# Opendigitalradio/ODR-AudioEnc

Hardware: AMD Instinct MI355X
Metric: real-time stereo DAB MP2 streams sustained (frames/s) @128 kbps/48 kHz (higher is better)
Workload: dtype f64; 1 GPU; 4096 streams/GPU x 48 kHz stereo (mode 's') x 128 kbps, psy 1, full encode (BASELINE configs[1]), 32 frames/stream/step; streams_per_gpu=4096, parallelism=streams sharded over 1 GPU(s), no data-path collective

## Files before the change

odr-audioenc_amd/csrc/mp2_pack.h:

```cpp
#ifndef MP2_WAVE_PARTS
#error "include mp2_wave.h"
#endif
struct TlFrameOut { uint8_t *bytes; uint32_t *words; uint8_t *scfcrc; };
template <int PSY, int NCH = 0>
TL_FN void tl_encode_frame(TlMainLds &w, const TlTables *TL_RESTRICT T, const TlBlockShared *TL_RESTRICT B,
                           const TlConfig *TL_RESTRICT C, const TlPsyOut *TL_RESTRICT PO,
                           const TlPcmView &pv, int xpad_len, const TlFrameOut &fo,
                           const double *TL_RESTRICT enw_s, const TlPackTables *TL_RESTRICT K, int padding, TlTaps *taps, long long *sp)
{
    constexpr int FB = TlMainLds::kFbBatch;
    const int nch = NCH ? NCH : C->nch, sblimit = C->sblimit;
    PA(double, smp, 36);
    PA(int, scf, 3);

    TL_STAMP(sp, 0);
    TL_PRIO2(TL_PS_FB);
    tl_filterbank(w, B, enw_s, nch, smp);

    TL_STAMP(sp, 1);
    TL_PRIO2(1);
#if !defined(TL_EMULATE) && TL_ENC_LEVEL >= 5
    for (int b = 0; b < 36; b++) TL_KEEP(smp[b]);
    scf[0] = scf[1] = scf[2] = 0;
#endif
    PV(int, a_ln); PV(int, a_nbal);
    TL_LANES_BEGIN
// ... 433 lines not shown
            int bytepos = i < xpad_len - 2 ? xstart + i : lg_frame - 2 + (i - (xpad_len - 2));
            tl_put_bits(frame, bytepos * 8, w.xpad[i], 8);
        }
    }
    TL_LANES_END

    } else {
        TL_LANES_BEGIN
        if (lane < 4) w.ncentre[lane] = 0;
        TL_LANES_END
    }
    if (taps) {
        TL_LANES_BEGIN
        const int c = lane & 1, sb = lane >> 1;
        taps->smr[c][sb] = (c < nch && (C->psy != 1 || sb < sblimit)) ? w.smr[c][sb] : 0.0;
        taps->scfsi[c][sb] = w.scfsi[c][sb]; taps->bit_alloc[c][sb] = w.balloc[c][sb];
        for (int gr = 0; gr < 3; gr++) taps->scalar[c][gr][sb] = w.scf[c][gr][sb];
        if (lane == 0) { taps->adb_left = adb_left; taps->mode = mode; taps->mode_ext = mode_ext; taps->jsbound = jsbound; taps->crc16 = (int)crc16; }
        if (lane < 4) taps->scfcrc[lane] = lane < C->dab_ext ? (uint8_t)w.ncentre[lane] : 0;
        TL_LANES_END
    }

    TL_STAMP(sp, 6);
    const int nwords = (lg_frame + 3) >> 2;
    TL_LANES_BEGIN
    for (int i = lane; i < nwords; i += 64) {
        if (fo.words) fo.words[i] = frame[i];
        else {
            const uint32_t le = tl_bswap(frame[i]);
            const int rem = lg_frame - 4 * i;
            if (rem >= 4) ((uint32_t *)fo.bytes)[i] = le;
            else for (int b = 0; b < rem; b++) fo.bytes[4 * i + b] = (uint8_t)(le >> (8 * b));
        }
    }
    if (lane < 4) fo.scfcrc[lane] = lane < C->dab_ext ? (uint8_t)w.ncentre[lane] : 0;
    TL_LANES_END
    TL_PRIO2(0);
    TL_STAMP(sp, 7);
}

template <int PSY>
TL_FN void tl_encode_pair(TlMainLds &w, const TlBlockShared *TL_RESTRICT B, const TlConfig *TL_RESTRICT C, const TlPsyOut *const (&PO)[2],
                          const int (&xpad_len)[2], const uint8_t *const (&xpad_src)[2], const TlFrameOut (&fo)[2],
                          const double *TL_RESTRICT enw_s, const TlPackTables *TL_RESTRICT K, const int (&padding)[2])
{
    const int sblimit = C->sblimit;
    const int padpk = padding[0] | (padding[1] << 1);
    PA(double, smp, 36);
    PA(int, scf, 3);
    TL_PRIO2(TL_PS_FB);
    tl_filterbank(w, B, enw_s, 2, smp);
    TL_PRIO2(1);
    TL_LANES_BEGIN
    const int c = lane & 1, sb = lane >> 1;
    if (sb < sblimit) {
        unsigned lo = 63;
        for (int gr = 0; gr < 3; gr++) {
            double m = fabs(L(smp)[gr * 12 + 11]);
            for (int j = 10; j >= 0; j--) { double t = fabs(L(smp)[gr * 12 + j]); if (t > m) m = t; }
// ... 234 lines not shown
        const int u = lane >> 5, l5 = lane & 31;
        if (l5 < C->dab_ext) {
            const int grp = C->dab_ext - 1 - l5;
            const unsigned c8 = ((grp == 0 ? c8g[0] : grp == 1 ? c8g[1] : grp == 2 ? c8g[2] : c8g[3]) >> (16 * u)) & 0xffu;
            const int tail = (u ? lg_frame[1] : lg_frame[0]) - 2 - C->dab_ext;
            tl_put_bits(w.u.frame[u], (tail + l5) * 8, c8, 8);
            w.ncentre[4 * u + l5] = (int16_t)c8;
        }
        TL_LANES_END
    }
#pragma unroll
    for (int u = 0; u < 2; u++)
        if (xpad_len[u]) {
            const int xl = xpad_len[u], xstart = lg_frame[u] - C->dab_ext - xl;
            TL_LANES_BEGIN
            for (int i = lane; i < xl; i += 64) {
                const int bytepos = i < xl - 2 ? xstart + i : lg_frame[u] - 2 + (i - (xl - 2));
                tl_put_bits(w.u.frame[u], bytepos * 8, xpad_src[u][i], 8);
            }
            TL_LANES_END
        }
#pragma unroll
    for (int u = 0; u < 2; u++) {
        const int nwords = (lg_frame[u] + 3) >> 2;
        const uint32_t *frame = w.u.frame[u];
        TL_LANES_BEGIN
        for (int i = lane; i < nwords; i += 64) {
            if (fo[u].words) fo[u].words[i] = frame[i];
            else {
                const uint32_t le = tl_bswap(frame[i]);
                const int rem = lg_frame[u] - 4 * i;
                if (rem >= 4) ((uint32_t *)fo[u].bytes)[i] = le;
                else for (int b = 0; b < rem; b++) fo[u].bytes[4 * i + b] = (uint8_t)(le >> (8 * b));
            }
        }
        if (lane < 4) fo[u].scfcrc[lane] = lane < C->dab_ext ? (uint8_t)w.ncentre[4 * u + lane] : 0;
        TL_LANES_END
    }
    TL_PRIO2(0);
}
```

odr-audioenc_amd/csrc/mp2_types.h:

```cpp
#pragma once
#include <stdint.h>

#define TL_MAX_FRAME_BYTES 1728
#define TL_MAX_FRAME_WORDS (TL_MAX_FRAME_BYTES / 4)
#define TL_HIST 480
#define TL_MAX_XPAD 256

struct TlBlockShared {
    double dbtable[1002];
    double scalefactor[64];
    double snr_line[9][16];
    int16_t bits12_line[9][16];
    uint16_t qinfo_line[9][16];
    double dct_t[16][2][16];
    uint8_t sfpat[32];
    double scale_db[64];
};

struct TlPackTables {
    double qa[18], qb[18];
    double steps2n_f[18];
    int32_t steps[18];
    int32_t steps2n[18];
    uint16_t crc_xpow[512];
// ... 104 lines not shown
    const int32_t *stream_cfg;
    const int32_t *stream_list;
    TlStreamState *state;
    const int16_t *pcm;
    const uint8_t *xpad;
    const int32_t *xpad_len;
    uint8_t *out;
    int32_t *out_len;
    TlTaps *taps;
    long long *stamps;
    const TlPsy2Tables *psy2_tables;
    TlPsy2State *psy2_state;
    TlPsyOut *psy_out;
    uint8_t *scfcrc;
    uint32_t *newpend;
    uint8_t *padbits;
    double *newlag;
    int32_t *work;
    const int32_t *partner;
    const int32_t *chain_list;
    int32_t nstreams, nframes, out_stride, nlist;
    int32_t nchain, p2_nwhole, p2_k, p2_plen;
    int32_t psy2_flip, pad_;
};
```

odr-audioenc_amd/csrc/mp2_units.h:

```cpp
#ifndef MP2_WAVE_PARTS
#error "include mp2_wave.h"
#endif
TL_FN int tl_cfg_index(const TlLaunch &A, int s) { return A.stream_cfg ? A.stream_cfg[s] : 0; }
TL_FN int tl_slot_step(double &lag, double frac)
{
    if (frac == 0) return 0;
    if (lag > (frac - 1.0)) { lag -= frac; return 0; }
    lag += (1 - frac);
    return 1;
}
TL_FN void tl_slots_stream(const TlLaunch &A, int s)
{
    const double frac = A.configs[tl_cfg_index(A, s)].pad_frac;
    double lag = A.state[s].slot_lag;
    for (int f = 0; f < A.nframes; f++) A.padbits[(size_t)f * (size_t)A.nstreams + (size_t)s] = (uint8_t)tl_slot_step(lag, frac);
    A.newlag[s] = lag;
}

TL_FN TlPcmView tl_pcm_view(const TlLaunch &A, const TlStreamState *st, int s, int f)
{
    const size_t slot = (size_t)f * (size_t)A.nstreams + (size_t)s;
    TlPcmView pv;
    pv.cur[0] = A.pcm + slot * 2304; pv.cur[1] = pv.cur[0] + 1152;
    pv.hist[0] = f == 0 ? &st->hist[0][0] : A.pcm + (slot - (size_t)A.nstreams) * 2304 + (1152 - TL_HIST);
// ... 119 lines not shown
#pragma unroll
        for (int c = 0; c < 2; c++) {
            if (c >= nch) break;
            uint64_t *d = (uint64_t *)&w.u.fbk.pcm[c][0];
#pragma unroll
            for (int it = 0; it < HT; it++) if (64 * it + 64 <= HP || lane < HP - 64 * it) d[lane + 64 * it] = vh[c][it];
#pragma unroll
            for (int it = 0; it < CT; it++) if (64 * it + 64 <= CP || lane < CP - 64 * it) d[HP + lane + 64 * it] = vc[c][it];
        }
    }
    TL_LANES_END
}
TL_FN int tl_stage_xpad(TlMainLds &w, const TlLaunch &A, const TlConfig *C, size_t slot)
{
    if (!A.xpad_len) return 0;
    int xl = A.xpad_len[slot];
    if (xl < 2 || xl > TL_MAX_XPAD || xl > C->dab_length) xl = 0;
    TL_LANES_BEGIN
    for (int i = lane; i < xl; i += 64) w.xpad[i] = A.xpad[slot * TL_MAX_XPAD + i];
    TL_LANES_END
    return xl;
}

template <int PSY, int NCH = 0>
TL_FN void tl_main_unit(TlMainLds &w, const TlBlockShared *TL_RESTRICT B, const double *TL_RESTRICT enw_s, const TlPackTables *TL_RESTRICT K, const TlLaunch &A, int s, int f, int ci = -1)
{
    const TlConfig *C = &A.configs[ci >= 0 ? ci : TL_UNI_I(tl_cfg_index(A, s))];
    TlStreamState *st = &A.state[s];
    const size_t slot = (size_t)f * (size_t)A.nstreams + (size_t)s;
    const TlPcmView pv = tl_pcm_view(A, st, s, f);
#ifdef TL_NO_MAIN_STAMPS
    long long *sp = nullptr;
#else
    long long *sp = A.stamps ? A.stamps + slot * 32 : nullptr;
#endif
    TL_STAMP(sp, 31);
    tl_stage_pcm(w, pv, NCH ? NCH : C->nch);
    const int xl = tl_stage_xpad(w, A, C, slot);
    TlFrameOut fo;
    fo.bytes = f + 1 < A.nframes ? A.out + (slot + (size_t)A.nstreams) * (size_t)A.out_stride : nullptr;
    fo.words = f + 1 < A.nframes ? nullptr : A.newpend + (size_t)s * TL_MAX_FRAME_WORDS;
    fo.scfcrc = A.scfcrc + slot * 4;
    const int padding = A.padbits ? (int)A.padbits[slot] : 0;
    tl_encode_frame<PSY, NCH>(w, A.tables, B, C, PSY == 2 ? &A.psy_out[slot] : nullptr, pv, xl, fo, enw_s, K, padding,
                                A.taps ? &A.taps[slot] : nullptr, sp);
}

template <int PSY>
TL_FN void tl_main_pair(TlMainLds &w, const TlBlockShared *TL_RESTRICT B, const double *TL_RESTRICT enw_s, const TlPackTables *TL_RESTRICT K, const TlLaunch &A, int s0, int s1, int f)
{
    const TlConfig *C = &A.configs[tl_cfg_index(A, s0)];
    const int ss[2] = {s0, s1};
    tl_stage_pcm(w, tl_pcm_view_pair(A, s0, s1, f), 2);
    TlFrameOut fo[2];
    const TlPsyOut *po[2];
    const uint8_t *xsrc[2];
    int xl[2], padding[2];
#pragma unroll
    for (int u = 0; u < 2; u++) {
        const size_t slot = (size_t)f * (size_t)A.nstreams + (size_t)ss[u];
        fo[u].bytes = f + 1 < A.nframes ? A.out + (slot + (size_t)A.nstreams) * (size_t)A.out_stride : nullptr;
        fo[u].words = f + 1 < A.nframes ? nullptr : A.newpend + (size_t)ss[u] * TL_MAX_FRAME_WORDS;
        fo[u].scfcrc = A.scfcrc + slot * 4;
        po[u] = PSY == 2 ? &A.psy_out[slot] : nullptr;
        padding[u] = A.padbits ? (int)A.padbits[slot] : 0;
        int x = A.xpad_len ? A.xpad_len[slot] : 0;
        if (x < 2 || x > TL_MAX_XPAD || x > C->dab_length) x = 0;
        xl[u] = x; xsrc[u] = A.xpad ? A.xpad + slot * TL_MAX_XPAD : nullptr;
    }
    tl_encode_pair<PSY>(w, B, C, po, xl, xsrc, fo, enw_s, K, padding);
}

union TlFrameLds { TlPsyLds p; TlMainLds m; };
template <int PSY, int NCH = 0>
TL_FN void tl_frame_unit(TlFrameLds &w, const double *TL_RESTRICT db, const TlBlockShared *TL_RESTRICT B, const double *TL_RESTRICT enw_s,
                         const TlPackTables *TL_RESTRICT K, const TlLaunch &Apsy, TL_KARG Amain_p, int s, int f, int s2 = -1)
{
    PA(double, rec, 4);
    int ci = -1;
    tl_psy_unit<PSY, NCH>(w.p, db, Apsy, s, f, rec, s2, &ci);
    TL_SYNC();
    TL_LAUNDER(Amain_p); TL_LAUNDER(s); TL_LAUNDER(f); TL_LAUNDER(s2); TL_LAUNDER(ci);
    const TlLaunch Amain = *Amain_p;
    TL_LANES_BEGIN
    if (lane < 32) {
        w.m.smr[0][lane] = L(rec)[0]; w.m.smr[1][lane] = L(rec)[1];
        w.m.psy_m[0][lane] = L(rec)[2]; w.m.psy_m[1][lane] = L(rec)[3];
    }
    TL_LANES_END
    if (s2 >= 0) tl_main_pair<TL_PSY_EXT>(w.m, B, enw_s, K, Amain, s, s2, f);
    else tl_main_unit<TL_PSY_EXT, NCH>(w.m, B, enw_s, K, Amain, s, f, ci);
}
// ... 59 lines not shown
```

odr-audioenc_amd/csrc/tlb_batch.cpp:

```cpp
#include "tlb_internal.h"
#include "tlb_plan.h"
#include "tl_libm.h"

extern "C" {

int tlb_device_count(void)
{
    int n = 0;
    if (hipGetDeviceCount(&n) != hipSuccess) return 0;
    return n;
}
int tlb_lds_bytes_per_stream(void) { return (int)tlk_lds_bytes_per_wave(); }
#define TLB_STR2(x) #x
#define TLB_STR(x) TLB_STR2(x)
const char *tlb_version(void)
{
    return "odr-audioenc_amd 0.5 (gfx950, a wavefront per (stream, frame), fp64, glibc 2.35 transcendentals; built with HIP "
           TLB_STR(HIP_VERSION_MAJOR) "." TLB_STR(HIP_VERSION_MINOR) "." TLB_STR(HIP_VERSION_PATCH) ", clang " __clang_version__ ", ISA guard passed)";
}

void tlb_destroy(tlb_batch *b)
{
    if (!b) return;
    (void)hipSetDevice(b->device);
// ... 85 lines not shown
        {
            const int longest = (b->h_configs[found].frame_bytes + (b->h_configs[found].pad_frac != 0 ? 1 : 0) + 3) & ~3;
            if (longest > b->out_stride) b->out_stride = longest;
        }
        {
            const int unit = 3 * b->h_configs[found].kbps, fb = b->h_configs[found].frame_bytes;
            if (fb % unit) b->max_upf = 0;
            else if (b->max_upf && fb / unit > b->max_upf) b->max_upf = fb / unit;
        }
    }
    HIPCHK(hipSetDevice(device));
    { int n = 0; if (hipDeviceGetAttribute(&n, hipDeviceAttributeMultiprocessorCount, device) == hipSuccess && n > 0) b->num_cu = n; }
    TlbMem &m = b->mem;
    TlTables *ht = new TlTables;
    tl_build_tables(ht);
    b->d_tables = m.scratch<TlTables>(1);
    m.upload(b->d_tables, ht, sizeof(TlTables));
    delete ht;
    b->cfg_cap = b->h_configs.size() + 8;
    HIPCHK(hipMalloc(&b->d_configs, sizeof(TlConfig) * b->cfg_cap));
    HIPCHK(hipMemcpy(b->d_configs, b->h_configs.data(), sizeof(TlConfig) * b->h_configs.size(), hipMemcpyHostToDevice));
    b->d_stream_cfg = m.scratch<int32_t>((size_t)nstreams);
    m.upload(b->d_stream_cfg, b->h_stream_cfg.data(), sizeof(int32_t) * (size_t)nstreams);
    b->d_state = m.dev<TlStreamState>((size_t)nstreams);
    b->h_gain.assign((size_t)nstreams, 1.0);
    b->d_gain = m.scratch<double>((size_t)nstreams);
    m.upload(b->d_gain, b->h_gain.data(), sizeof(double) * (size_t)nstreams);
    b->d_newpend = m.dev<uint32_t>(TL_MAX_FRAME_WORDS * (size_t)nstreams);
    b->d_work = m.scratch<int32_t>(TL_HEAD_STRIDE * 9);
    MEMCHK(m);
    if (int rc = batch_build_lists(b)) return rc;
    HIPCHK(hipEventCreate(&b->ev0));
    HIPCHK(hipEventCreate(&b->ev1));
    HIPCHK(hipEventCreate(&b->ev_mid));
    return TLB_OK;
}

tlb_batch *tlb_create(int device, int nstreams, const tlb_stream_config *cfgs, int *err)
{
    if (nstreams <= 0 || !cfgs) { if (err) *err = TLB_ERR_ARG; return nullptr; }
    tlb_batch *b = new tlb_batch;
    int rc = tlb_create_impl(b, device, nstreams, cfgs);
    if (err) *err = rc;
    if (rc) { tlb_destroy(b); return nullptr; }
    return b;
}

static int batch_clear_streams(tlb_batch *b, int s0, int n)
{
    HIPCHK(hipMemset(b->d_state + s0, 0, sizeof(TlStreamState) * (size_t)n));
    if (b->d_psy2_state) HIPCHK(hipMemset(b->d_psy2_state + 2 * (size_t)s0, 0, sizeof(TlPsy2State) * 2 * (size_t)n));
    HIPCHK(hipMemset(b->d_newpend + (size_t)s0 * TL_MAX_FRAME_WORDS, 0, sizeof(uint32_t) * TL_MAX_FRAME_WORDS * (size_t)n));
    if (b->d_newlag) HIPCHK(hipMemset(b->d_newlag + s0, 0, sizeof(double) * (size_t)n));
    if (b->d_edi_state_tmp) HIPCHK(hipMemset(b->d_edi_state_tmp + s0, 0, sizeof(TlEdiState) * (size_t)n));
    if (b->d_pseq_tmp) HIPCHK(hipMemset(b->d_pseq_tmp + s0, 0, sizeof(uint16_t) * (size_t)n));
    if (b->d_dec_state) HIPCHK(hipMemset(b->d_dec_state + s0, 0, sizeof(TlDecStream) * (size_t)n));
    if (b->d_cmp_hist) HIPCHK(hipMemset(b->d_cmp_hist + (size_t)s0 * 2 * TL_CMP_HIST, 0, sizeof(int16_t) * 2 * TL_CMP_HIST * (size_t)n));
    if (int rc = feed_clear_streams(b, s0, n)) return rc;
    if (int rc = feed_down_clear_streams(b, s0, n)) return rc;
    if (int rc = resample_clear_streams(b, s0, n)) return rc;
    return decimate_clear_streams(b, s0, n);
}

static int meters_clear_streams(tlb_batch *b, int s0, int n)
{
    if (int rc = loudness_clear_streams(b, s0, n)) return rc;
    return truepeak_clear_streams(b, s0, n);
}

int tlb_reset(tlb_batch *b)
{
    if (!b) return TLB_ERR_ARG;
    HIPCHK(hipSetDevice(b->device));
    HIPCHK(hipDeviceSynchronize());
    HIPCHK(hipMemcpy(b->d_configs, b->h_configs.data(), sizeof(TlConfig) * b->h_configs.size(), hipMemcpyHostToDevice));
    HIPCHK(hipMemcpy(b->d_stream_cfg, b->h_stream_cfg.data(), sizeof(int32_t) * (size_t)b->nstreams, hipMemcpyHostToDevice));
    if (int rc = batch_build_lists(b)) return rc;
    if (int rc = batch_clear_streams(b, 0, b->nstreams)) return rc;
    if (int rc = meters_clear_streams(b, 0, b->nstreams)) return rc;
    b->frames = 0; b->psy2_flip = 0; b->work_clean = false; b->broken = false;
    return TLB_OK;
}

int tlb_stream_reset(tlb_batch *b, int stream)
{
    if (!b || stream < 0 || stream >= b->nstreams) return TLB_ERR_ARG;
    HIPCHK(hipSetDevice(b->device));
    HIPCHK(hipDeviceSynchronize());
    if (int rc = meters_clear_streams(b, stream, 1)) return rc;
    return batch_clear_streams(b, stream, 1);
}

int tlb_stream_finish(tlb_batch *b, int stream, uint8_t *out, size_t out_size)
{
    if (!b || stream < 0 || stream >= b->nstreams || (!out && out_size)) return -TLB_ERR_ARG;
    if (hipSetDevice(b->device) != hipSuccess || hipDeviceSynchronize() != hipSuccess) return -TLB_ERR_HIP;
    TlStreamState *st = new TlStreamState;
    hipError_t e = hipMemcpy(st, b->d_state + stream, sizeof(TlStreamState), hipMemcpyDeviceToHost);
    int n = 0;
    if (e == hipSuccess && st->frames_done > 0) {
        n = st->pending_len;
        if ((size_t)n > out_size) n = (int)out_size;
        for (int i = 0; i < n; i++) out[i] = (uint8_t)(st->pending[i >> 2] >> (24 - 8 * (i & 3)));
    }
    delete st;
    if (e != hipSuccess) return -TLB_ERR_HIP;
    if (int rc = batch_clear_streams(b, stream, 1)) return -rc;
    return n;
}

int tlb_stream_reconfigure(tlb_batch *b, int stream, const tlb_stream_config *cfg)
{
    if (!b || !cfg || stream < 0 || stream >= b->nstreams) return TLB_ERR_ARG;
    int found = tlb_find_config(b->h_uniq, *cfg);
    TlConfig c;
    if (found < 0) { if (int rc = tl_build_config(&c, cfg->samplerate, cfg->mode, cfg->bitrate, cfg->psy_model, cfg->pad_len)) return rc; }
    else c = b->h_configs[(size_t)found];
    if (!resample_rate_fits(b, stream, cfg->samplerate) || !decimate_rate_fits(b, stream, cfg->samplerate)) return TLB_ERR_SAMPLERATE;
    if (((c.frame_bytes + (c.pad_frac != 0 ? 1 : 0) + 3) & ~3) > b->out_stride) return TLB_ERR_ARG;
    {
        const int unit = 3 * c.kbps, upf = c.frame_bytes % unit ? 0 : c.frame_bytes / unit;
// ... 41 lines not shown
int tlb_nstreams(const tlb_batch *b) { return b ? b->nstreams : 0; }
int tlb_frame_bytes(const tlb_batch *b, int s) { return (b && s >= 0 && s < b->nstreams) ? b->h_configs[b->h_stream_cfg[s]].frame_bytes : 0; }
int tlb_out_stride(const tlb_batch *b) { return b ? b->out_stride : 0; }
long tlb_frames_encoded(const tlb_batch *b) { return b ? b->frames : 0; }
#ifdef TLB_FAULT_INJECT
int tlb_debug_fail_next(tlb_batch *b, int nth) { if (!b || nth < 0) return TLB_ERR_ARG; b->fail_in = nth; return TLB_OK; }
int tlb_debug_alloc_fail_next(int nth) { if (nth < 0) return TLB_ERR_ARG; TlbMem::fail_in.store(nth); return TLB_OK; }
#endif

}
int tlb_launch(tlb_batch *b, const int16_t *d_pcm, int nframes, const uint8_t *d_xpad, const int32_t *d_xpad_len,
               uint8_t *d_out, TlTaps *d_taps, hipStream_t st, long long *d_stamps, int32_t *d_out_len)
{
    if (!b || !d_pcm || !d_out || nframes <= 0) return TLB_ERR_ARG;
    for (int p = 0; p < 4; p++) if ((long)b->n_list[p] * nframes > (1L << 30)) return TLB_ERR_ARG;
    if (b->broken) { fprintf(stderr, "libtoolame-dab-hip: a launch or a reconfiguration of this batch failed half way; tlb_reset() it before encoding on\n"); return TLB_ERR_HIP; }
    HIPCHK(hipSetDevice(b->device));
    struct Guard { tlb_batch *b; int flip; bool ok; ~Guard() { if (!ok) { b->psy2_flip = flip; b->work_clean = false; b->broken = true; } } } guard_{b, b->psy2_flip, false};
#ifdef TLB_FAULT_INJECT
    if (b->fail_in > 0 && --b->fail_in == 0) { fprintf(stderr, "libtoolame-dab-hip: injected fault (tlb_debug_fail_next)\n"); return TLB_ERR_HIP; }
#endif
    TlLaunch A;
    memset(&A, 0, sizeof A);
    A.tables = b->d_tables; A.configs = b->d_configs; A.stream_cfg = b->h_configs.size() == 1 ? nullptr : b->d_stream_cfg; A.state = b->d_state;
    A.pcm = d_pcm; A.xpad = d_xpad_len ? d_xpad : nullptr; A.xpad_len = d_xpad ? d_xpad_len : nullptr;
    A.out = d_out; A.out_len = d_out_len; A.taps = d_taps; A.stamps = d_stamps;
    A.psy2_tables = b->d_psy2_tables; A.psy2_state = b->d_psy2_state; A.partner = b->d_partner;
    A.nstreams = b->nstreams; A.nframes = nframes; A.out_stride = b->out_stride;
    {
        if (b->n_list[2]) HIPCHK(stage_reserve(b, TLB_STAGE_PSY_OUT, (size_t)nframes * (size_t)b->nstreams * sizeof(TlPsyOut)));
        HIPCHK(stage_reserve(b, TLB_STAGE_SCFCRC, (size_t)nframes * (size_t)b->nstreams * 4));
        A.psy_out = (TlPsyOut *)b->stage[TLB_STAGE_PSY_OUT]; A.scfcrc = (uint8_t *)b->stage[TLB_STAGE_SCFCRC]; A.newpend = b->d_newpend; A.work = b->d_work;
        if (b->pads[0] || b->pads[1] || b->pads[2] || b->pads[3]) HIPCHK(stage_reserve(b, TLB_STAGE_PADBITS, (size_t)nframes * (size_t)b->nstreams));
    }
    HIPCHK(hipEventRecord(b->ev0, st));
    b->have_mid = false;
    for (int p = 0; p < 4; p++) {
        if (!b->n_list[p]) continue;
        A.stream_list = b->n_list[p] == b->nstreams ? nullptr : b->d_list[p]; A.nlist = b->n_list[p];
        const long units = (long)b->n_list[p] * nframes;
        A.padbits = b->pads[p] ? (uint8_t *)b->stage[TLB_STAGE_PADBITS] : nullptr; A.newlag = b->d_newlag;
        if (b->pads[p]) HIPCHK(tlk_slots((unsigned)((b->n_list[p] + 255) / 256), st, A));
        if (!b->work_clean) HIPCHK(hipMemsetAsync(b->d_work, 0, sizeof(int32_t) * TL_HEAD_STRIDE * 9, st));
        b->work_clean = false;
        long qb = 0;
        if (p == 2) {
            A.chain_list = b->d_chain; A.nchain = b->n_chain; A.psy2_flip = b->psy2_flip;
            const int nunits = tl_psy2_plan(b->n_chain, nframes, b->num_cu * TL_PSY2_WAVES, &A.p2_nwhole, &A.p2_k, &A.p2_plen);
            qb = ((long)nunits + TL_PSY2_WAVES - 1) / TL_PSY2_WAVES;
            if (qb > b->num_cu) qb = b->num_cu;
        }
        if (p == 1 || p == 3) {
            long mb1 = (units + TL_MAIN_WAVES - 1) / TL_MAIN_WAVES;
            if (mb1 > b->num_cu) mb1 = b->num_cu;
            const bool pr = b->list_pairs[p] && !d_taps && !d_stamps;
            HIPCHK(tlk_frame(p, pr, b->list_stereo[p], (unsigned)mb1, st, A));
            HIPCHK(tlk_finish((unsigned)((b->n_list[p] + 3) / 4), st, A));
            b->work_clean = true;
            continue;
        }
        if (p == 2) HIPCHK(tlk_psy2((unsigned)qb, st, A));
        if (p == 2 && b->n_list[p] == b->nstreams) { HIPCHK(hipEventRecord(b->ev_mid, st)); b->have_mid = true; }
        long mb = (units + TL_MAIN_WAVES - 1) / TL_MAIN_WAVES;
        if (mb > b->num_cu) mb = b->num_cu;
        const bool pr = b->list_pairs[p] && !d_taps && !d_stamps;
        HIPCHK(tlk_main(p, pr, b->list_stereo[p], (unsigned)mb, st, A));
        HIPCHK(tlk_finish((unsigned)((b->n_list[p] + 3) / 4), st, A));
        b->work_clean = true;
    }
    HIPCHK(hipEventRecord(b->ev1, st));
    if (b->n_list[2]) b->psy2_flip ^= 1;
    guard_.ok = true;
    b->last_stream = st; b->timed = true;
    b->frames += nframes;
    return TLB_OK;
}

extern "C" {

int tlb_encode_device(tlb_batch *b, const int16_t *d_pcm, int nframes, const uint8_t *d_xpad, const int32_t *d_xpad_len,
                      uint8_t *d_out, void *hip_stream)
{
    return tlb_launch(b, d_pcm, nframes, d_xpad, d_xpad_len, d_out, nullptr, (hipStream_t)hip_stream);
}
int tlb_encode_device_len(tlb_batch *b, const int16_t *d_pcm, int nframes, const uint8_t *d_xpad, const int32_t *d_xpad_len,
                          uint8_t *d_out, int32_t *d_out_len, void *hip_stream)
{
    return tlb_launch(b, d_pcm, nframes, d_xpad, d_xpad_len, d_out, nullptr, (hipStream_t)hip_stream, nullptr, d_out_len);
}

int tlb_encode_host(tlb_batch *b, const int16_t *pcm, int nframes, const uint8_t *xpad, const int32_t *xpad_len,
                    uint8_t *out, void *taps)
{
    return tlb_encode_host_len(b, pcm, nframes, xpad, xpad_len, out, nullptr, taps);
// ... 80 lines not shown
    HIPCHK(hipMemcpy(d_pcm, pcm, slots * 2304 * sizeof(int16_t), hipMemcpyHostToDevice));
    int rc = tlb_launch(b, d_pcm, nframes, nullptr, nullptr, d_out, nullptr, nullptr, d_st);
    HIPCHK(hipDeviceSynchronize());
    HIPCHK(hipMemcpy(stamps, d_st, slots * 32 * sizeof(long long), hipMemcpyDeviceToHost));

    return rc;
}

int tlb_zmq_msg_stride(const tlb_batch *b) { return b ? 12 + b->out_stride : 0; }
int tlb_egress_unit_bytes(const tlb_batch *b, int s) { return (b && s >= 0 && s < b->nstreams) ? 3 * b->h_configs[b->h_stream_cfg[s]].kbps : 0; }
int tlb_egress_units_per_frame(const tlb_batch *b, int s)
{
    if (!b || s < 0 || s >= b->nstreams) return 0;
    const TlConfig &c = b->h_configs[b->h_stream_cfg[s]];
    return c.frame_bytes % (3 * c.kbps) ? 0 : c.frame_bytes / (3 * c.kbps);
}
int tlb_egress_max_units_per_frame(const tlb_batch *b) { return b ? b->max_upf : 0; }


int tlb_flush_device_len(tlb_batch *b, uint8_t *d_out, int32_t *d_out_len, void *hip_stream)
{
    if (!b || !d_out) return TLB_ERR_ARG;
    HIPCHK(hipSetDevice(b->device));
    HIPCHK(tlk_flush((unsigned)b->nstreams, (hipStream_t)hip_stream, b->d_state, b->d_configs, b->d_stream_cfg, d_out, d_out_len, b->nstreams, b->out_stride));
    return TLB_OK;
}
int tlb_flush_device(tlb_batch *b, uint8_t *d_out, void *hip_stream) { return tlb_flush_device_len(b, d_out, nullptr, hip_stream); }

int tlb_flush_host_len(tlb_batch *b, uint8_t *out, int32_t *out_len)
{
    if (!b || !out) return TLB_ERR_ARG;
    HIPCHK(hipSetDevice(b->device));
    const size_t n = (size_t)b->nstreams * (size_t)b->out_stride;
    TlbMem m;
    uint8_t *d = m.scratch<uint8_t>(n); int32_t *dl = m.scratch<int32_t>((size_t)b->nstreams);
    MEMCHK(m);
    int rc = tlb_flush_device_len(b, d, dl, nullptr);
    hipError_t e = hipDeviceSynchronize();
    if (e == hipSuccess) e = hipMemcpy(out, d, n, hipMemcpyDeviceToHost);
    if (e == hipSuccess && out_len) e = hipMemcpy(out_len, dl, sizeof(int32_t) * (size_t)b->nstreams, hipMemcpyDeviceToHost);
    if (e != hipSuccess) return TLB_ERR_HIP;
    return rc;
}
int tlb_flush_host(tlb_batch *b, uint8_t *out) { return tlb_flush_host_len(b, out, nullptr); }

int tlb_reference_send_schedule(const tlb_stream_config *cfg, int ncalls, int32_t *units_sent)
{
// ... 63 lines not shown
```

odr-audioenc_amd/csrc/tlb_internal.h:

```cpp
#pragma once
#include <hip/hip_runtime_api.h>
#include <math.h>
#include <stdio.h>
#include <stdlib.h>
#include <string.h>

#include <deque>
#include <memory>
#include <vector>

#include "../../include/toolame_batch.h"
#include "mp2_host.h"
#include "tl_kernels.h"
#include "tlb_inputs.h"
#include "tlb_mem.h"

static_assert(TL_MAX_XPAD == TLB_MAX_XPAD, "xpad record size");
#define TLB_HOST_CHUNKS 4

enum TlbStage {
    TLB_STAGE_PCM, TLB_STAGE_OUT, TLB_STAGE_XPAD, TLB_STAGE_XPAD_LEN, TLB_STAGE_TAPS,
    TLB_STAGE_PSY_OUT, TLB_STAGE_SCFCRC, TLB_STAGE_PADBITS,
    TLB_STAGE_OUT_LEN,
    TLB_STAGE_INGEST_IN, TLB_STAGE_INGEST_OUT, TLB_STAGE_INGEST_PEAKS,
// ... 56 lines not shown
            HIPCHK(hipDeviceSynchronize());
            std::unique_ptr<TlbMem> m(new TlbMem);
            tlb_frame_report *nr = m->scratch<tlb_frame_report>(slots);
            if (m->failed()) return TLB_ERR_HIP;
            rep_mem.swap(m);
            d_rep = nr; rep_slots = slots;
        }
        *d_report = d_rep;
        return TLB_OK;
    }
};

struct tlb_batch {
    int device = 0, nstreams = 0, out_stride = 0;
    long frames = 0;
    std::vector<TlConfig> h_configs;
    std::vector<tlb_stream_config> h_uniq;
    size_t cfg_cap = 0;
    std::vector<int32_t> h_stream_cfg;
    TlTables *d_tables = nullptr;
    TlConfig *d_configs = nullptr;
    int32_t *d_stream_cfg = nullptr;
    TlStreamState *d_state = nullptr;
    double *d_gain = nullptr;
    std::vector<double> h_gain;
    int32_t *d_list[4] = {nullptr, nullptr, nullptr, nullptr};
    int n_list[4] = {0, 0, 0, 0};
    TlPsy2Tables *d_psy2_tables = nullptr;
    TlPsy2State *d_psy2_state = nullptr;
    int psy2_flip = 0;
    int32_t *d_partner = nullptr;
    int32_t *d_chain = nullptr;
    int n_chain = 0;
    uint8_t *d_edi_version = nullptr;
    char h_edi_version[TL_EDI_MAX_VERSION] = {};
    int edi_version_len = -1;
    int32_t *d_frame_bytes = nullptr, *d_unit_bytes = nullptr;
    int max_upf = 1;
    TlEdiState *d_edi_state_tmp = nullptr;
    uint16_t *d_pseq_tmp = nullptr;
    hipEvent_t ev0 = nullptr, ev1 = nullptr, ev_mid = nullptr;
    bool have_mid = false;
    hipStream_t last_stream = nullptr;
    bool timed = false;
    void *stage[TLB_STAGE_COUNT] = {};
    size_t stage_cap[TLB_STAGE_COUNT] = {};
    hipStream_t s_in = nullptr, s_run = nullptr, s_out = nullptr;
    hipEvent_t ev_in[TLB_HOST_CHUNKS] = {}, ev_run[TLB_HOST_CHUNKS] = {};
    uint32_t *d_newpend = nullptr;
    double *d_newlag = nullptr;
    bool pads[4] = {false, false, false, false};
    bool list_pairs[4] = {false, false, false, false};
    bool list_stereo[4] = {false, false, false, false};
    int32_t *d_work = nullptr;
    bool work_clean = false;
    bool broken = false;
    int num_cu = 256;
    TlSynthTables *d_synth = nullptr;
    TlDecStream *d_dec_state = nullptr;
    uint8_t *d_dec_prev = nullptr;
    unsigned long long *d_dec_bad = nullptr;
    int16_t *d_cmp_hist = nullptr;
    uint32_t *d_rs_state = nullptr;
    int32_t *d_rs_ratio = nullptr;
    int16_t *d_rs_taps = nullptr;
    int rs_flip = 0;
    std::vector<long> rs_rate;
    std::vector<int32_t> rs_ratio, rs_pos;
    uint32_t *d_dc_state = nullptr;
    int32_t *d_dc_ratio = nullptr;
    int16_t *d_dc_taps = nullptr;
    int dc_flip = 0;
    std::vector<long> dc_rate;
    std::vector<int32_t> dc_ratio, dc_pos;
    FeedTable feed;
    std::unique_ptr<TlbMem> feed_prev_mem;
    int32_t *d_feed_cfg = nullptr;
// ... 111 lines not shown
```

odr-audioenc_amd/csrc/toolame_hip.hip:

```cpp
#include <hip/hip_runtime.h>
#include <stdio.h>
#include <stdlib.h>
#include <math.h>
#include <string.h>

#include "../../include/toolame_batch.h"
#include "mp2_host.h"
#include "mp2_wave.h"
#include "tl_kernel_util.h"
#include "tl_kernels.h"

static_assert(TL_MAX_XPAD == TLB_MAX_XPAD, "xpad record size");


#define TL_LIST_BLOCK_LOG2 5
static __device__ __forceinline__ bool tl_take_unit(int32_t *heads, int nlist, int nframes, int grp, int &hop, int &k, int &f, int first)
{
    const int nunits = nlist * nframes, nblocks = (nunits + (1 << TL_LIST_BLOCK_LOG2) - 1) >> TL_LIST_BLOCK_LOG2;
    while (hop < 8) {
        const int q = (grp + hop) & 7;
        const int lim = ((nblocks - q + 7) >> 3) << TL_LIST_BLOCK_LOG2;
        const int ng = (((int)gridDim.x - q + 7) >> 3) * (int)(blockDim.x >> 6);
        int v;
        if (first >= 0) { v = first; first = -1; }
        else {
            if (hop > 0 && ng + __hip_atomic_load(&heads[q * TL_HEAD_STRIDE], __ATOMIC_RELAXED, __HIP_MEMORY_SCOPE_AGENT) >= lim) { hop++; continue; }
            v = ng + tl_next_unit(&heads[q * TL_HEAD_STRIDE]);
        }
        if (v >= lim) { hop++; continue; }
        const int u = ((((v >> TL_LIST_BLOCK_LOG2) << 3) + q) << TL_LIST_BLOCK_LOG2) + (v & ((1 << TL_LIST_BLOCK_LOG2) - 1));
        if (u >= nunits) continue;
        k = u / nframes; f = u - k * nframes;
        return true;
    }
    return false;
}

__global__ void tl_psy2_kernel(TlLaunch A);
struct TlMainShared { double enw_s[512]; char bytes[sizeof(TlBlockShared) - offsetof(TlBlockShared, scalefactor)]; TlPackTables pack; };
static_assert(offsetof(TlBlockShared, dbtable) == 0 && offsetof(TlBlockShared, scalefactor) == sizeof(double) * 1002, "dbtable leads TlBlockShared");
static_assert((sizeof(TlMainShared) + TL_MAIN_WAVES * sizeof(TlMainLds) + TL_LDS_GRANULE - 1) / TL_LDS_GRANULE <= 128, "the encode workgroup fits a CU");
static_assert(sizeof(TlPackTables) % 8 == 0, "copied as doubles");
template <int PSY, bool PAIRS, int NCH = 0>
__global__ void __launch_bounds__(64 * TL_MAIN_WAVES) __attribute__((amdgpu_waves_per_eu(TL_MAIN_WPE, TL_MAIN_WPE))) tl_main_kernel(TlLaunch A)
{
    __shared__ TlMainShared sh;
    __shared__ TlMainLds lds[TL_MAIN_WAVES];
    TL_ENCODE_PROLOGUE(sh, A.tables, (void)0);
    TlMainLds &wl = lds[wave_v];
    for (int hop = 0, k, f, first = ((int)blockIdx.x >> 3) * TL_MAIN_WAVES + wave; tl_take_unit(A.work + TL_HEAD_STRIDE, A.nlist, A.nframes, grp, hop, k, f, first); first = -1) {
        const int s = A.stream_list ? __builtin_amdgcn_readfirstlane(A.stream_list[k]) : k;
        if constexpr (PAIRS) {
            int s2;
            if (!tl_unit_partner(A, s, s2)) continue;
            s2 = __builtin_amdgcn_readfirstlane(s2);
            if (s2 >= 0) { tl_main_pair<PSY>(wl, B, sh.enw_s, &sh.pack, A, s, s2, f); continue; }
        }
        tl_main_unit<PSY, NCH>(wl, B, sh.enw_s, &sh.pack, A, s, f);
    }
}

static_assert((sizeof(double) * 1258 + sizeof(TlMainShared) + TL_MAIN_WAVES * sizeof(TlFrameLds) + TL_LDS_GRANULE - 1) / TL_LDS_GRANULE <= 128, "the workgroup fits a CU");
template <int PSY, bool PAIRS, int NCH = 0>
__global__ void __launch_bounds__(64 * TL_MAIN_WAVES) __attribute__((amdgpu_waves_per_eu(TL_MAIN_WPE, TL_MAIN_WPE))) tl_frame_kernel(TlLaunch A)
{
    __shared__ __attribute__((aligned(16))) double dbt[1258];
    __shared__ TlMainShared sh;
    __shared__ TlFrameLds lds[TL_MAIN_WAVES];
    TL_ENCODE_PROLOGUE(sh, A.tables, for (int i = (int)threadIdx.x; i < 1258; i += 64 * TL_MAIN_WAVES) dbt[i] = A.tables->dblog[i]);
    TlFrameLds &wl = lds[wave_v];
    for (int hop = 0, k, f, first = ((int)blockIdx.x >> 3) * TL_MAIN_WAVES + wave; tl_take_unit(A.work + TL_HEAD_STRIDE, A.nlist, A.nframes, grp, hop, k, f, first); first = -1) {
        const int s = A.stream_list ? __builtin_amdgcn_readfirstlane(A.stream_list[k]) : k;
#if defined(__HIP_DEVICE_COMPILE__)
        TlKArg a1 = (TlKArg)__builtin_amdgcn_kernarg_segment_ptr(), a2 = a1;
        asm volatile("" : "+s"(a1));
        const TlLaunch A1 = *a1;
        if constexpr (PAIRS) {
            int s2;
            if (!tl_unit_partner(A, s, s2)) continue;
            tl_frame_unit<PSY>(wl, dbt, B, sh.enw_s, &sh.pack, A1, a2, s, f, __builtin_amdgcn_readfirstlane(s2));
        } else tl_frame_unit<PSY, NCH>(wl, dbt, B, sh.enw_s, &sh.pack, A1, a2, s, f);
#endif
    }
}

__global__ void __launch_bounds__(256) tl_slots_kernel(TlLaunch A)
{
    const int k = (int)(blockIdx.x * 256 + threadIdx.x);
    if (k >= A.nlist) return;
    tl_slots_stream(A, A.stream_list ? A.stream_list[k] : k);
}

__global__ void __launch_bounds__(256) tl_finish_kernel(TlLaunch A)
// ... 58 lines not shown
```

Before: 36.85 million frames/s.

## Fold finish kernel into main encode kernel with double-buffered stream state

Removes the separate finish kernel launch when taps/stamps are off. The main/frame kernels now write the pending-frame fixups, out_len, history and next-step stream state directly into a second (ping-pong) TlStreamState buffer. The scfcrc bytes are patched into the previous frame's output via a stored base pointer instead of a later pass. Work-queue heads are also double-buffered, with the idle set zeroed inside the kernel so the next step needs no memset. This trades one kernel launch and its global round-trip for extra per-unit work, doubled state memory and more complex cross-frame pointer logic.

```diff
diff --git a/odr-audioenc_amd/csrc/mp2_pack.h b/odr-audioenc_amd/csrc/mp2_pack.h
--- a/odr-audioenc_amd/csrc/mp2_pack.h
+++ b/odr-audioenc_amd/csrc/mp2_pack.h
@@ -2,6 +2,29 @@
 #error "include mp2_wave.h"
 #endif
 struct TlFrameOut { uint8_t *bytes; uint32_t *words; uint8_t *scfcrc; };
+TL_FN void tl_emit_frame(const TlFrameOut &fo, const uint32_t *frame, int len, int dab_ext, const int16_t *scratch, int u)
+{
+    if (!fo.scfcrc) {
+        TL_LANES_BEGIN
+        if (lane < dab_ext) {
+            const uint64_t base = ((const uint64_t *)(scratch + 16))[u];
+            if (base) ((uint8_t *)(uintptr_t)base)[len - dab_ext + lane] = (uint8_t)scratch[4 * u + lane];
+        }
+        TL_LANES_END
+    }
+    if (fo.words) {
+        TL_LANES_BEGIN
+        for (int i = lane; i < ((len + 3) >> 2); i += 64) fo.words[i] = frame[i];
+        TL_LANES_END
+        return;
+    }
+    const int h1 = fo.scfcrc ? len : len - 2, h0 = h1 - (fo.scfcrc ? 0 : dab_ext), wfull = h0 >> 2;
+    TL_LANES_BEGIN
+    for (int i = lane; i < wfull; i += 64) ((uint32_t *)fo.bytes)[i] = tl_bswap(frame[i]);
+    const int p = 4 * wfull + lane;
+    if (p < len && (p < h0 || p >= h1)) fo.bytes[p] = ((const uint8_t *)frame)[p ^ 3];
+    TL_LANES_END
+}
 template <int PSY, int NCH = 0>
 TL_FN void tl_encode_frame(TlMainLds &w, const TlTables *TL_RESTRICT T, const TlBlockShared *TL_RESTRICT B,
                            const TlConfig *TL_RESTRICT C, const TlPsyOut *TL_RESTRICT PO,
@@ -481,19 +504,12 @@
     }
 
     TL_STAMP(sp, 6);
-    const int nwords = (lg_frame + 3) >> 2;
-    TL_LANES_BEGIN
-    for (int i = lane; i < nwords; i += 64) {
-        if (fo.words) fo.words[i] = frame[i];
-        else {
-            const uint32_t le = tl_bswap(frame[i]);
-            const int rem = lg_frame - 4 * i;
-            if (rem >= 4) ((uint32_t *)fo.bytes)[i] = le;
-            else for (int b = 0; b < rem; b++) fo.bytes[4 * i + b] = (uint8_t)(le >> (8 * b));
-        }
-    }
-    if (lane < 4) fo.scfcrc[lane] = lane < C->dab_ext ? (uint8_t)w.ncentre[lane] : 0;
-    TL_LANES_END
+    tl_emit_frame(fo, frame, lg_frame, C->dab_ext, w.ncentre, 0);
+    if (fo.scfcrc) {
+        TL_LANES_BEGIN
+        if (lane < 4) fo.scfcrc[lane] = lane < C->dab_ext ? (uint8_t)w.ncentre[lane] : 0;
+        TL_LANES_END
+    }
     TL_PRIO2(0);
     TL_STAMP(sp, 7);
 }
@@ -774,20 +790,12 @@
         }
 #pragma unroll
     for (int u = 0; u < 2; u++) {
-        const int nwords = (lg_frame[u] + 3) >> 2;
-        const uint32_t *frame = w.u.frame[u];
-        TL_LANES_BEGIN
-        for (int i = lane; i < nwords; i += 64) {
-            if (fo[u].words) fo[u].words[i] = frame[i];
-            else {
-                const uint32_t le = tl_bswap(frame[i]);
-                const int rem = lg_frame[u] - 4 * i;
-                if (rem >= 4) ((uint32_t *)fo[u].bytes)[i] = le;
-                else for (int b = 0; b < rem; b++) fo[u].bytes[4 * i + b] = (uint8_t)(le >> (8 * b));
-            }
-        }
-        if (lane < 4) fo[u].scfcrc[lane] = lane < C->dab_ext ? (uint8_t)w.ncentre[4 * u + lane] : 0;
-        TL_LANES_END
+        tl_emit_frame(fo[u], w.u.frame[u], lg_frame[u], C->dab_ext, w.ncentre, u);
+        if (fo[u].scfcrc) {
+            TL_LANES_BEGIN
+            if (lane < 4) fo[u].scfcrc[lane] = lane < C->dab_ext ? (uint8_t)w.ncentre[4 * u + lane] : 0;
+            TL_LANES_END
+        }
     }
     TL_PRIO2(0);
 }
diff --git a/odr-audioenc_amd/csrc/mp2_types.h b/odr-audioenc_amd/csrc/mp2_types.h
--- a/odr-audioenc_amd/csrc/mp2_types.h
+++ b/odr-audioenc_amd/csrc/mp2_types.h
@@ -150,4 +150,6 @@
     int32_t nstreams, nframes, out_stride, nlist;
     int32_t nchain, p2_nwhole, p2_k, p2_plen;
     int32_t psy2_flip, pad_;
+    TlStreamState *fold_out;
+    int32_t *work_zero;
 };
diff --git a/odr-audioenc_amd/csrc/mp2_units.h b/odr-audioenc_amd/csrc/mp2_units.h
--- a/odr-audioenc_amd/csrc/mp2_units.h
+++ b/odr-audioenc_amd/csrc/mp2_units.h
@@ -165,6 +165,84 @@
     return xl;
 }
 
+#ifdef TL_EMULATE
+static long tl_emu_fold_units = 0;
+#endif
+TL_FN void tl_fold_begin(TlMainLds &w, const TlLaunch &A, const TlConfig *C, int s, int f, int s2, int padding0, int padding1)
+{
+    uint64_t base[2] = {0, 0};
+    for (int u = 0; u < 2; u++) {
+        const int su = u ? s2 : s, padding = u ? padding1 : padding0;
+        if (su < 0) break;
+#ifdef TL_EMULATE
+        tl_emu_fold_units++;
+#endif
+        const size_t slot = (size_t)f * (size_t)A.nstreams + (size_t)su;
+        const TlStreamState *in = &A.state[su];
+        uint8_t *o = A.out + slot * (size_t)A.out_stride;
+        if (f > 0) {
+            const int prevpad = A.padbits ? (int)A.padbits[slot - (size_t)A.nstreams] : 0;
+            base[u] = (uint64_t)(uintptr_t)o + (uint64_t)(int64_t)(prevpad - padding - 2);
+            if (A.out_len) {
+                const int len = C->frame_bytes + prevpad;
+                TL_LANES_BEGIN
+                if (lane == 0) A.out_len[slot] = len;
+                TL_LANES_END
+            }
+        } else {
+            constexpr int T = (TL_MAX_FRAME_WORDS + 63) / 64;
+            PA(uint32_t, v, T);
+            TL_LANES_BEGIN
+#pragma unroll
+            for (int t = 0; t < T; t++) { L(v)[t] = 0; if (4 * (lane + 64 * t) < A.out_stride) L(v)[t] = in->pending[lane + 64 * t]; }
+            TL_LANES_END
+            const int len = in->frames_done > 0 ? in->pending_len : 0;
+            const int h1 = len - 2, h0 = h1 - C->dab_ext;
+            TL_LANES_BEGIN
+#pragma unroll
+            for (int t = 0; t < T; t++) {
+                const int p = 4 * (lane + 64 * t);
+                const uint32_t le = tl_bswap(L(v)[t]);
+                if (p + 4 <= len && (p + 4 <= h0 || p >= h1)) *(uint32_t *)(o + p) = le;
+                else for (int b = 0; b < 4; b++) if (p + b < len && (p + b < h0 || p + b >= h1)) o[p + b] = (uint8_t)(le >> (8 * b));
+            }
+            if (lane == 0 && A.out_len) A.out_len[slot] = len;
+            TL_LANES_END
+            if (len) base[u] = (uint64_t)(uintptr_t)o + (uint64_t)(int64_t)(len - 2 - (C->frame_bytes + padding));
+        }
+        if (f + 1 < A.nframes) continue;
+        TlStreamState *out = &A.fold_out[su];
+        const int16_t *last = A.pcm + slot * 2304;
+        constexpr int HP = TL_HIST / 4;
+        PA(uint64_t, hv, 4);
+        TL_LANES_BEGIN
+#pragma unroll
+        for (int q = 0; q < 4; q++) { L(hv)[q] = 0; if (lane + 64 * (q & 1) < HP) L(hv)[q] = ((const uint64_t *)(last + (q >> 1) * 1152 + (1152 - TL_HIST)))[lane + 64 * (q & 1)]; }
+        TL_LANES_END
+        const int nch = C->nch;
+        TL_LANES_BEGIN
+#pragma unroll
+        for (int q = 0; q < 4; q++) if (lane + 64 * (q & 1) < HP) ((uint64_t *)&out->hist[q >> 1][0])[lane + 64 * (q & 1)] = (q >> 1) < nch ? L(hv)[q] : 0ull;
+        if (lane == 0) {
+            out->frames_done = in->frames_done + A.nframes; out->pending_len = C->frame_bytes + padding;
+            out->slot_lag = A.padbits ? A.newlag[su] : in->slot_lag;
+        }
+        TL_LANES_END
+    }
+    TL_LANES_BEGIN
+    if (lane == 0) { uint64_t *k = (uint64_t *)&w.ncentre[16]; k[0] = base[0]; k[1] = base[1]; }
+    TL_LANES_END
+}
+TL_FN TlFrameOut tl_frame_out(const TlLaunch &A, int s, int f)
+{
+    const size_t slot = (size_t)f * (size_t)A.nstreams + (size_t)s;
+    TlFrameOut fo;
+    fo.bytes = f + 1 < A.nframes ? A.out + (slot + (size_t)A.nstreams) * (size_t)A.out_stride : nullptr;
+    fo.words = f + 1 < A.nframes ? nullptr : A.fold_out ? &A.fold_out[s].pending[0] : A.newpend + (size_t)s * TL_MAX_FRAME_WORDS;
+    fo.scfcrc = A.fold_out ? nullptr : A.scfcrc + slot * 4;
+    return fo;
+}
+
 template <int PSY, int NCH = 0>
 TL_FN void tl_main_unit(TlMainLds &w, const TlBlockShared *TL_RESTRICT B, const double *TL_RESTRICT enw_s, const TlPackTables *TL_RESTRICT K, const TlLaunch &A, int s, int f, int ci = -1)
 {
@@ -180,11 +258,10 @@
     TL_STAMP(sp, 31);
     tl_stage_pcm(w, pv, NCH ? NCH : C->nch);
     const int xl = tl_stage_xpad(w, A, C, slot);
-    TlFrameOut fo;
-    fo.bytes = f + 1 < A.nframes ? A.out + (slot + (size_t)A.nstreams) * (size_t)A.out_stride : nullptr;
-    fo.words = f + 1 < A.nframes ? nullptr : A.newpend + (size_t)s * TL_MAX_FRAME_WORDS;
-    fo.scfcrc = A.scfcrc + slot * 4;
+    const TlFrameOut fo = tl_frame_out(A, s, f);
     const int padding = A.padbits ? (int)A.padbits[slot] : 0;
+    const bool fold = A.fold_out != nullptr;
+    if (fold) tl_fold_begin(w, A, C, s, f, -1, padding, 0);
     tl_encode_frame<PSY, NCH>(w, A.tables, B, C, PSY == 2 ? &A.psy_out[slot] : nullptr, pv, xl, fo, enw_s, K, padding,
                                 A.taps ? &A.taps[slot] : nullptr, sp);
 }
@@ -202,15 +279,15 @@
 #pragma unroll
     for (int u = 0; u < 2; u++) {
         const size_t slot = (size_t)f * (size_t)A.nstreams + (size_t)ss[u];
-        fo[u].bytes = f + 1 < A.nframes ? A.out + (slot + (size_t)A.nstreams) * (size_t)A.out_stride : nullptr;
-        fo[u].words = f + 1 < A.nframes ? nullptr : A.newpend + (size_t)ss[u] * TL_MAX_FRAME_WORDS;
-        fo[u].scfcrc = A.scfcrc + slot * 4;
+        fo[u] = tl_frame_out(A, ss[u], f);
         po[u] = PSY == 2 ? &A.psy_out[slot] : nullptr;
         padding[u] = A.padbits ? (int)A.padbits[slot] : 0;
         int x = A.xpad_len ? A.xpad_len[slot] : 0;
         if (x < 2 || x > TL_MAX_XPAD || x > C->dab_length) x = 0;
         xl[u] = x; xsrc[u] = A.xpad ? A.xpad + slot * TL_MAX_XPAD : nullptr;
     }
+    const bool fold = A.fold_out != nullptr;
+    if (fold) tl_fold_begin(w, A, C, s0, f, s1, padding[0], padding[1]);
     tl_encode_pair<PSY>(w, B, C, po, xl, xsrc, fo, enw_s, K, padding);
 }
 
diff --git a/odr-audioenc_amd/csrc/tlb_batch.cpp b/odr-audioenc_amd/csrc/tlb_batch.cpp
--- a/odr-audioenc_amd/csrc/tlb_batch.cpp
+++ b/odr-audioenc_amd/csrc/tlb_batch.cpp
@@ -131,12 +131,12 @@
     HIPCHK(hipMemcpy(b->d_configs, b->h_configs.data(), sizeof(TlConfig) * b->h_configs.size(), hipMemcpyHostToDevice));
     b->d_stream_cfg = m.scratch<int32_t>((size_t)nstreams);
     m.upload(b->d_stream_cfg, b->h_stream_cfg.data(), sizeof(int32_t) * (size_t)nstreams);
-    b->d_state = m.dev<TlStreamState>((size_t)nstreams);
+    b->d_state = m.dev<TlStreamState>(2 * (size_t)nstreams);
     b->h_gain.assign((size_t)nstreams, 1.0);
     b->d_gain = m.scratch<double>((size_t)nstreams);
     m.upload(b->d_gain, b->h_gain.data(), sizeof(double) * (size_t)nstreams);
     b->d_newpend = m.dev<uint32_t>(TL_MAX_FRAME_WORDS * (size_t)nstreams);
-    b->d_work = m.scratch<int32_t>(TL_HEAD_STRIDE * 9);
+    b->d_work = m.scratch<int32_t>(TL_HEAD_STRIDE * 9 * 2);
     MEMCHK(m);
     if (int rc = batch_build_lists(b)) return rc;
     HIPCHK(hipEventCreate(&b->ev0));
@@ -157,7 +157,7 @@
 
 static int batch_clear_streams(tlb_batch *b, int s0, int n)
 {
-    HIPCHK(hipMemset(b->d_state + s0, 0, sizeof(TlStreamState) * (size_t)n));
+    for (int c = 0; c < 2; c++) HIPCHK(hipMemset(b->d_state + (size_t)c * (size_t)b->nstreams + s0, 0, sizeof(TlStreamState) * (size_t)n));
     if (b->d_psy2_state) HIPCHK(hipMemset(b->d_psy2_state + 2 * (size_t)s0, 0, sizeof(TlPsy2State) * 2 * (size_t)n));
     HIPCHK(hipMemset(b->d_newpend + (size_t)s0 * TL_MAX_FRAME_WORDS, 0, sizeof(uint32_t) * TL_MAX_FRAME_WORDS * (size_t)n));
     if (b->d_newlag) HIPCHK(hipMemset(b->d_newlag + s0, 0, sizeof(double) * (size_t)n));
@@ -187,7 +187,7 @@
     if (int rc = batch_build_lists(b)) return rc;
     if (int rc = batch_clear_streams(b, 0, b->nstreams)) return rc;
     if (int rc = meters_clear_streams(b, 0, b->nstreams)) return rc;
-    b->frames = 0; b->psy2_flip = 0; b->work_clean = false; b->broken = false;
+    b->frames = 0; b->psy2_flip = 0; b->state_flip = 0; b->work_set = 0; b->work_clean = false; b->broken = false;
     return TLB_OK;
 }
 
@@ -205,7 +205,7 @@
     if (!b || stream < 0 || stream >= b->nstreams || (!out && out_size)) return -TLB_ERR_ARG;
     if (hipSetDevice(b->device) != hipSuccess || hipDeviceSynchronize() != hipSuccess) return -TLB_ERR_HIP;
     TlStreamState *st = new TlStreamState;
-    hipError_t e = hipMemcpy(st, b->d_state + stream, sizeof(TlStreamState), hipMemcpyDeviceToHost);
+    hipError_t e = hipMemcpy(st, b->cur_state() + stream, sizeof(TlStreamState), hipMemcpyDeviceToHost);
     int n = 0;
     if (e == hipSuccess && st->frames_done > 0) {
         n = st->pending_len;
@@ -293,7 +293,7 @@
 #endif
     TlLaunch A;
     memset(&A, 0, sizeof A);
-    A.tables = b->d_tables; A.configs = b->d_configs; A.stream_cfg = b->h_configs.size() == 1 ? nullptr : b->d_stream_cfg; A.state = b->d_state;
+    A.tables = b->d_tables; A.configs = b->d_configs; A.stream_cfg = b->h_configs.size() == 1 ? nullptr : b->d_stream_cfg; A.state = b->cur_state();
     A.pcm = d_pcm; A.xpad = d_xpad_len ? d_xpad : nullptr; A.xpad_len = d_xpad ? d_xpad_len : nullptr;
     A.out = d_out; A.out_len = d_out_len; A.taps = d_taps; A.stamps = d_stamps;
     A.psy2_tables = b->d_psy2_tables; A.psy2_state = b->d_psy2_state; A.partner = b->d_partner;
@@ -301,9 +301,11 @@
     {
         if (b->n_list[2]) HIPCHK(stage_reserve(b, TLB_STAGE_PSY_OUT, (size_t)nframes * (size_t)b->nstreams * sizeof(TlPsyOut)));
         HIPCHK(stage_reserve(b, TLB_STAGE_SCFCRC, (size_t)nframes * (size_t)b->nstreams * 4));
-        A.psy_out = (TlPsyOut *)b->stage[TLB_STAGE_PSY_OUT]; A.scfcrc = (uint8_t *)b->stage[TLB_STAGE_SCFCRC]; A.newpend = b->d_newpend; A.work = b->d_work;
+        A.psy_out = (TlPsyOut *)b->stage[TLB_STAGE_PSY_OUT]; A.scfcrc = (uint8_t *)b->stage[TLB_STAGE_SCFCRC]; A.newpend = b->d_newpend;
         if (b->pads[0] || b->pads[1] || b->pads[2] || b->pads[3]) HIPCHK(stage_reserve(b, TLB_STAGE_PADBITS, (size_t)nframes * (size_t)b->nstreams));
     }
+    const bool fold = !d_taps && !d_stamps;
+    if (fold) A.fold_out = b->d_state + (size_t)(1 - b->state_flip) * (size_t)b->nstreams;
     HIPCHK(hipEventRecord(b->ev0, st));
     b->have_mid = false;
     for (int p = 0; p < 4; p++) {
@@ -312,8 +314,10 @@
         const long units = (long)b->n_list[p] * nframes;
         A.padbits = b->pads[p] ? (uint8_t *)b->stage[TLB_STAGE_PADBITS] : nullptr; A.newlag = b->d_newlag;
         if (b->pads[p]) HIPCHK(tlk_slots((unsigned)((b->n_list[p] + 255) / 256), st, A));
-        if (!b->work_clean) HIPCHK(hipMemsetAsync(b->d_work, 0, sizeof(int32_t) * TL_HEAD_STRIDE * 9, st));
+        if (!b->work_clean) HIPCHK(hipMemsetAsync(b->d_work, 0, sizeof(int32_t) * TL_HEAD_STRIDE * 9 * 2, st));
         b->work_clean = false;
+        A.work = b->d_work + (size_t)b->work_set * TL_HEAD_STRIDE * 9;
+        A.work_zero = fold ? b->d_work + (size_t)(1 - b->work_set) * TL_HEAD_STRIDE * 9 : nullptr;
         long qb = 0;
         if (p == 2) {
             A.chain_list = b->d_chain; A.nchain = b->n_chain; A.psy2_flip = b->psy2_flip;
@@ -326,7 +330,8 @@
             if (mb1 > b->num_cu) mb1 = b->num_cu;
             const bool pr = b->list_pairs[p] && !d_taps && !d_stamps;
             HIPCHK(tlk_frame(p, pr, b->list_stereo[p], (unsigned)mb1, st, A));
-            HIPCHK(tlk_finish((unsigned)((b->n_list[p] + 3) / 4), st, A));
+            if (fold) b->work_set ^= 1;
+            else HIPCHK(tlk_finish((unsigned)((b->n_list[p] + 3) / 4), st, A));
             b->work_clean = true;
             continue;
         }
@@ -336,11 +341,13 @@
         if (mb > b->num_cu) mb = b->num_cu;
         const bool pr = b->list_pairs[p] && !d_taps && !d_stamps;
         HIPCHK(tlk_main(p, pr, b->list_stereo[p], (unsigned)mb, st, A));
-        HIPCHK(tlk_finish((unsigned)((b->n_list[p] + 3) / 4), st, A));
+        if (fold) b->work_set ^= 1;
+        else HIPCHK(tlk_finish((unsigned)((b->n_list[p] + 3) / 4), st, A));
         b->work_clean = true;
     }
     HIPCHK(hipEventRecord(b->ev1, st));
     if (b->n_list[2]) b->psy2_flip ^= 1;
+    if (fold) b->state_flip ^= 1;
     guard_.ok = true;
     b->last_stream = st; b->timed = true;
     b->frames += nframes;
@@ -467,7 +474,7 @@
 {
     if (!b || !d_out) return TLB_ERR_ARG;
     HIPCHK(hipSetDevice(b->device));
-    HIPCHK(tlk_flush((unsigned)b->nstreams, (hipStream_t)hip_stream, b->d_state, b->d_configs, b->d_stream_cfg, d_out, d_out_len, b->nstreams, b->out_stride));
+    HIPCHK(tlk_flush((unsigned)b->nstreams, (hipStream_t)hip_stream, b->cur_state(), b->d_configs, b->d_stream_cfg, d_out, d_out_len, b->nstreams, b->out_stride));
     return TLB_OK;
 }
 int tlb_flush_device(tlb_batch *b, uint8_t *d_out, void *hip_stream) { return tlb_flush_device_len(b, d_out, nullptr, hip_stream); }
diff --git a/odr-audioenc_amd/csrc/tlb_internal.h b/odr-audioenc_amd/csrc/tlb_internal.h
--- a/odr-audioenc_amd/csrc/tlb_internal.h
+++ b/odr-audioenc_amd/csrc/tlb_internal.h
@@ -102,6 +102,8 @@
     TlConfig *d_configs = nullptr;
     int32_t *d_stream_cfg = nullptr;
     TlStreamState *d_state = nullptr;
+    int state_flip = 0;
+    TlStreamState *cur_state() const { return d_state + (size_t)state_flip * (size_t)nstreams; }
     double *d_gain = nullptr;
     std::vector<double> h_gain;
     int32_t *d_list[4] = {nullptr, nullptr, nullptr, nullptr};
@@ -133,6 +135,7 @@
     bool list_pairs[4] = {false, false, false, false};
     bool list_stereo[4] = {false, false, false, false};
     int32_t *d_work = nullptr;
+    int work_set = 0;
     bool work_clean = false;
     bool broken = false;
     int num_cu = 256;
diff --git a/odr-audioenc_amd/csrc/toolame_hip.hip b/odr-audioenc_amd/csrc/toolame_hip.hip
--- a/odr-audioenc_amd/csrc/toolame_hip.hip
+++ b/odr-audioenc_amd/csrc/toolame_hip.hip
@@ -36,6 +36,8 @@
     return false;
 }
 
+#define TL_ZERO_OTHER_HEADS(A) do { if ((A).work_zero && blockIdx.x == 0 && threadIdx.x < 9) (A).work_zero[threadIdx.x * TL_HEAD_STRIDE] = 0; } while (0)
+
 __global__ void tl_psy2_kernel(TlLaunch A);
 struct TlMainShared { double enw_s[512]; char bytes[sizeof(TlBlockShared) - offsetof(TlBlockShared, scalefactor)]; TlPackTables pack; };
 static_assert(offsetof(TlBlockShared, dbtable) == 0 && offsetof(TlBlockShared, scalefactor) == sizeof(double) * 1002, "dbtable leads TlBlockShared");
@@ -48,6 +50,7 @@
     __shared__ TlMainLds lds[TL_MAIN_WAVES];
     TL_ENCODE_PROLOGUE(sh, A.tables, (void)0);
     TlMainLds &wl = lds[wave_v];
+    TL_ZERO_OTHER_HEADS(A);
     for (int hop = 0, k, f, first = ((int)blockIdx.x >> 3) * TL_MAIN_WAVES + wave; tl_take_unit(A.work + TL_HEAD_STRIDE, A.nlist, A.nframes, grp, hop, k, f, first); first = -1) {
         const int s = A.stream_list ? __builtin_amdgcn_readfirstlane(A.stream_list[k]) : k;
         if constexpr (PAIRS) {
@@ -69,6 +72,7 @@
     __shared__ TlFrameLds lds[TL_MAIN_WAVES];
     TL_ENCODE_PROLOGUE(sh, A.tables, for (int i = (int)threadIdx.x; i < 1258; i += 64 * TL_MAIN_WAVES) dbt[i] = A.tables->dblog[i]);
     TlFrameLds &wl = lds[wave_v];
+    TL_ZERO_OTHER_HEADS(A);
     for (int hop = 0, k, f, first = ((int)blockIdx.x >> 3) * TL_MAIN_WAVES + wave; tl_take_unit(A.work + TL_HEAD_STRIDE, A.nlist, A.nframes, grp, hop, k, f, first); first = -1) {
         const int s = A.stream_list ? __builtin_amdgcn_readfirstlane(A.stream_list[k]) : k;
 #if defined(__HIP_DEVICE_COMPILE__)
```

Measured after the change: 36.84 million frames/s (median of 3 runs). Within noise of the previous version (-0.0%).
